# Dunni3/keypoint-diffusion

Measured on AMD Instinct MI355X. Metric: denoising steps/sec, higher is better.
Workload: dtype f32; 1 GPU; egnn_all_atom dynamics (6 EGNN layers, hidden 256, update_kp_feat; fixed receptor encoder), batch of 64 synthetic 300-atom pockets / 25-atom ligands per GPU, T=500, seeded random-init weights, every step taken from the t=T ligand state; batch_per_gpu=64, n_rec=300, n_lig=25, parallelism=dp1

## Files before the change

### keypoint-diffusion_amd/csrc/egnn.hip

```cpp
#include <string.h>

#include <map>
#include <set>
#include <string>
#include <vector>

#include "egnn_kernels.h"
#include "egnn_wide.h"
#include "mfma_core.h"

using namespace kpd;

namespace {

struct LayerW {
    float *wp_e[4], *wx_e[4], *b_e[4], *wr_e[4], *watt[4];
    float *wp_c[4], *wx_c[4], *b_c[4], *wr_c[4], *w3[4];
    void *wh_e[4], *wh_c[4];
    void *chh_p[2][NSLOT];
    void *wh_a[2], *wh_b[2], *wh_2[2];
    float *wp_p[2][NSLOT], *wx_p[2][NSLOT], *b_p[2][NSLOT];
    float *ch_p[2][NSLOT], *wcol_p[2][NSLOT];
    float *wp_a[2], *wx_a[2], *wp_b[2], *wx_b[2], *b0[2], *wp_2[2], *wx_2[2], *b2[2], *ln_w[2], *ln_b[2];
};

const int kSrcNt[4] = {NT_LIG, NT_KP, NT_LIG, NT_KP};
const int kDstNt[4] = {NT_LIG, NT_LIG, NT_KP, NT_KP};
const int kSrcSlot[4] = {0, 0, 6, 4};
const int kDstSlot[4] = {2, 4, 2, 6};
const char *kEtName[4] = {"ll", "kl", "lk", "kk"};
const char *kNtName[2] = {"lig", "kp"};

std::vector<std::string> split(const std::string &s, char c) {
    std::vector<std::string> out;
    size_t p = 0;
    while (true) {
        size_t q = s.find(c, p);
        out.push_back(s.substr(p, q == std::string::npos ? q : q - p));
        if (q == std::string::npos) break;
        p = q + 1;
    }
    return out;
}

int et_index(const std::string &s) {
    for (int i = 0; i < 4; ++i)
        if (s == kEtName[i]) return i;
    return -1;
}
int nt_index(const std::string &s) {
    for (int i = 0; i < 2; ++i)
        if (s == kNtName[i]) return i;
    return -1;
}

}

struct kpd_egnn {
    kpd_egnn_config cfg;
    int n_et;
    int n_upd;
    bool rec_identity;
    Arena warena, ws;
    std::vector<LayerW> L;
    float *le_W0, *le_b0, *le_W1t, *le_b1;
    float *re_W0, *re_b0, *re_W1t, *re_b1;
    float *de_W0, *de_b0, *de_W1, *de_b1;
    std::set<std::string> expected, loaded;
    bool committed = false;
    int debug_layers = -1;
    bool f16_ok = true;
    float *widen_buf = nullptr;
    int *widen_map = nullptr;
    size_t widen_floats = 0, widen_ints = 0;
    int gemm_mode = 0;
    bool f32_only = false;
    int prune_last = 1;
    bool prof_on = false;
    std::vector<hipEvent_t> prof_ev;
    size_t prof_used = 0;

    int cap_B = 0, cap_lig = 0, cap_kp = 0, cap_kk = 0, cap_ll = 0, cap_kl = 0, cap_maxlig = 0, cap_maxkp = 0;
    int tile_cap = 0, tiles_et_cap[4] = {0, 0, 0, 0};
    float *h[2], *x[2], *P[2];
    float *hn_main[4], *hn_cont[4], *xn_main[4], *xn_cont[4];
    int *bidx[2];
    float *z[2];
    int *meta, *ll_deg, *ll_off, *kl_off, *kl_pg;
    kpd_lig_graph lg;
    EgnnWide *wide = nullptr;
};

static kpd_status build_weight_arena(kpd_egnn *m) {
    const kpd_egnn_config &c = m->cfg;
    m->warena.poison_at = 2;
    m->L.assign(c.n_layers, LayerW());
    return carve(m->warena, ARENA_TAIL, [&](Carve &A) {
        for (int i = 0; i < c.n_layers; ++i) {
            LayerW &w = m->L[i];
            const std::string pre = "egnn.conv_layers." + std::to_string(i) + ".";
            for (int et = 0; et < m->n_et; ++et) {
                A(w.wp_e[et], WP_FLOATS); A(w.wx_e[et], HS); A(w.b_e[et], HS); A(w.wr_e[et], HS); A(w.watt[et], HS);
                A(w.wp_c[et], WP_FLOATS); A(w.wx_c[et], HS); A(w.b_c[et], HS); A(w.wr_c[et], HS); A(w.w3[et], HS);
                A.as<unsigned short>(w.wh_e[et], WH_HALVES); A.as<unsigned short>(w.wh_c[et], WH_HALVES);
                for (int var = 0; var < 2; ++var) {
                    const int ss = kSrcSlot[et] + var, ds = kDstSlot[et] + var;
                    A(w.wp_p[kSrcNt[et]][ss], WP_FLOATS); A(w.wx_p[kSrcNt[et]][ss], HS);
                    A(w.wp_p[kDstNt[et]][ds], WP_FLOATS); A(w.wx_p[kDstNt[et]][ds], HS); A(w.b_p[kDstNt[et]][ds], HS);
                    A(w.ch_p[kSrcNt[et]][ss], 16 * 4096); A(w.wcol_p[kSrcNt[et]][ss], HS);
                    A(w.ch_p[kDstNt[et]][ds], 16 * 4096); A(w.wcol_p[kDstNt[et]][ds], HS);
                    A.as<unsigned short>(w.chh_p[kSrcNt[et]][ss], CHH_HALVES);
                    A.as<unsigned short>(w.chh_p[kDstNt[et]][ds], CHH_HALVES);
                }
                const std::string e = kEtName[et];
                for (const char *blk : {"edge_mlp.", "coord_mlp."})
                    for (const char *s : {".0.weight", ".0.bias", ".2.weight", ".2.bias"}) m->expected.insert(pre + blk + e + s);
                m->expected.insert(pre + "coord_mlp." + e + ".4.weight");
                m->expected.insert(pre + "soft_attention." + e + ".0.weight");
                m->expected.insert(pre + "soft_attention." + e + ".0.bias");
            }
            for (int nt = 0; nt < m->n_upd; ++nt) {
                A(w.wp_a[nt], WP_FLOATS); A(w.wx_a[nt], HS); A(w.wp_b[nt], WP_FLOATS); A(w.wx_b[nt], HS); A(w.b0[nt], HS);
                A(w.wp_2[nt], WP_FLOATS); A(w.wx_2[nt], HS); A(w.b2[nt], HS); A(w.ln_w[nt], HS); A(w.ln_b[nt], HS);
                A.as<unsigned short>(w.wh_a[nt], WH_HALVES); A.as<unsigned short>(w.wh_b[nt], WH_HALVES);
                A.as<unsigned short>(w.wh_2[nt], WH_HALVES);
                const std::string n = kNtName[nt];
                for (const char *s : {".0.weight", ".0.bias", ".2.weight", ".2.bias"}) m->expected.insert(pre + "node_mlp." + n + s);
                if (c.norm) {
                    m->expected.insert(pre + "layer_norm." + n + ".weight");
                    m->expected.insert(pre + "layer_norm." + n + ".bias");
// ... 468 lines not shown
        ea.use_tanh = c.use_tanh; ea.coords_range = c.coords_range;
        ea.tile_rows = tr;
        ea.gemm_mode = tr == TM ? m->gemm_mode : 0;
        for (int et = 0; et < 4; ++et) {
            ea.src[et] = esrc[et]; ea.dst[et] = edst[et];
            ea.src_nt[et] = kSrcNt[et]; ea.dst_nt[et] = kDstNt[et]; ea.src_slot[et] = kSrcSlot[et]; ea.dst_slot[et] = kDstSlot[et];
            ea.wr_e[et] = L.wr_e[et]; ea.wr_c[et] = L.wr_c[et];
            ea.wp_e[et] = L.wp_e[et]; ea.wx_e[et] = L.wx_e[et]; ea.b_e[et] = L.b_e[et];
            ea.wp_c[et] = L.wp_c[et]; ea.wx_c[et] = L.wx_c[et]; ea.b_c[et] = L.b_c[et];
            ea.wh_e[et] = L.wh_e[et]; ea.wh_c[et] = L.wh_c[et];
            ea.watt[et] = L.watt[et]; ea.w3[et] = L.w3[et];
            ea.hn_main[et] = m->hn_main[et]; ea.hn_cont[et] = m->hn_cont[et];
            ea.xn_main[et] = m->xn_main[et]; ea.xn_cont[et] = m->xn_cont[et];
        }
        const bool prof = m->prof_on && m->prof_used + 2 <= m->prof_ev.size();
        if (prof) KPD_HIP(hipEventRecord(m->prof_ev[m->prof_used], st));
        KPD_TRY(launch_egnn_edge(ea, last ? tile_cap_last : tile_cap, st));
        if (prof) {
            KPD_HIP(hipEventRecord(m->prof_ev[m->prof_used + 1], st));
            m->prof_used += 2;
        }
        auto fill_update = [&](NodeArgs &na, int nt) {
            na.n = n[nt]; na.h = m->h[nt]; na.x = m->x[nt]; na.bidx = m->bidx[nt]; na.z = m->z[nt];
            int k = 0;
            for (int et = 0; et < m->n_et; ++et)
                if (kDstNt[et] == nt && ((layer_etmask(li) >> et) & 1)) {
                    na.rowptr[k] = rowptr[et];
                    na.hn_main[k] = m->hn_main[et]; na.hn_cont[k] = m->hn_cont[et];
                    na.xn_main[k] = m->xn_main[et]; na.xn_cont[k] = m->xn_cont[et];
                    ++k;
                }
            na.n_in = k;
            na.wp_a = L.wp_a[nt]; na.wx_a = L.wx_a[nt]; na.wp_b = L.wp_b[nt]; na.wx_b = L.wx_b[nt]; na.b0 = L.b0[nt];
            na.wp_2 = L.wp_2[nt]; na.wx_2 = L.wx_2[nt]; na.b2 = L.b2[nt]; na.ln_w = L.ln_w[nt]; na.ln_b = L.ln_b[nt];
            na.ln_inv_n = 1.0f / (float)(c.hidden_nf + 1); na.ln_pad = (float)(HID - c.hidden_nf);
            na.wh_a = L.wh_a[nt]; na.wh_b = L.wh_b[nt]; na.wh_2 = L.wh_2[nt];
            na.norm = c.norm;
            na.tile_shift = 6;
        };
        {
            NodeLayerPair lp;
            memset(&lp, 0, sizeof(lp));
            for (int nt = 0; nt < 2; ++nt) {
                NodeLayerArgs &na = lp.nt[nt];
                na.u.n = n[nt]; na.u.h = m->h[nt];
                if (nt < m->n_upd && !(nt == NT_KP && last && prune)) {
                    fill_update(na.u, nt);
                    na.do_update = 1;
                }
                if (!na.do_update && !na.do_proj) na.u.n = 0;
            }
            lp.tiles0 = cdiv(lp.nt[0].u.n, TN);
            lp.gemm_mode = m->gemm_mode;
            KPD_TRY(launch_node_layer(lp, st));
        }
    }
    KPD_TRY(launch_decode(m->h[NT_LIG], m->x[NT_LIG], bt->lig_x, bt->n_lig, c.atom_nf, 2 * c.atom_nf, m->de_W0, m->de_b0,
                          m->de_W1, m->de_b1, eps_h, eps_x, st));
    return KPD_OK;
}

extern "C" kpd_status kpd_egnn_debug_state(kpd_egnn *m, const char *what, float *out, int64_t n_floats, void *stream) {
    KPD_REQUIRE(m && what && out, KPD_ERR_INVALID, "null argument");
    hipStream_t st = static_cast<hipStream_t>(stream);
    if (m->wide) return wide_debug_state(m->wide, what, out, n_floats, st);
    const std::string w(what);
    const float *src = nullptr;
    if (w == "h_lig") src = m->h[0];
    else if (w == "h_kp") src = m->h[1];
    else if (w == "x_lig") src = m->x[0];
    else if (w == "x_kp") src = m->x[1];
    else if (w == "z_lig") src = m->z[0];
    else if (w == "z_kp") src = m->z[1];
    else if (w.size() == 4 && (w.rfind("xnm", 0) == 0 || w.rfind("xnc", 0) == 0 || w.rfind("hnm", 0) == 0 || w.rfind("hnc", 0) == 0) &&
             w[3] >= '0' && w[3] < '4') {
        const int et = w[3] - '0';
        src = w[0] == 'x' ? (w[2] == 'm' ? m->xn_main[et] : m->xn_cont[et]) : (w[2] == 'm' ? m->hn_main[et] : m->hn_cont[et]);
    }
    else if (w.rfind("layers=", 0) == 0) {
        m->debug_layers = atoi(w.c_str() + 7);
        return KPD_OK;
    } else if (w.rfind("prune=", 0) == 0) {
        m->prune_last = atoi(w.c_str() + 6);
        return KPD_OK;
    } else if (w.rfind("gemm=", 0) == 0) {
        const std::string v = w.substr(5);
        KPD_REQUIRE(v == "f32" || v == "f16x2", KPD_ERR_INVALID, "gemm mode must be f32 or f16x2");
        KPD_REQUIRE(v == "f32" || !m->f32_only, KPD_ERR_INVALID,
                    "gemm=f16x2: atom_nf = %d / rec_nf = %d (hidden_nf = %d) run the exact fp32 path only; the f16x2 mode covers atom_nf <= 32 "
                    "with rec_nf <= 128 or 256, or the identity keypoint encoder at hidden_nf 256", m->cfg.atom_nf, m->cfg.rec_nf, m->cfg.hidden_nf);
        KPD_REQUIRE(v == "f32" || !m->committed || m->f16_ok, KPD_ERR_WEIGHTS, "%s", F16_RANGE_ERROR);
        m->gemm_mode = v == "f16x2" ? 1 : 0;
        return KPD_OK;
    }
    KPD_REQUIRE(src, KPD_ERR_INVALID, "unknown debug tap '%s'", what);
    KPD_HIP(hipMemcpyAsync(out, src, (size_t)n_floats * 4, hipMemcpyDeviceToDevice, st));
    return KPD_OK;
}

extern "C" kpd_status kpd_egnn_profile(kpd_egnn *m, int32_t enable) {
    KPD_REQUIRE(m, KPD_ERR_INVALID, "null handle");
    KPD_REQUIRE(!m->wide, KPD_ERR_INVALID, "kpd_egnn_profile times the fused edge kernel of hidden_nf <= 256; hidden_nf = %d has none",
                m->cfg.hidden_nf);
    if (enable && m->prof_ev.empty()) {
        m->prof_ev.resize(2 * 8192);
        for (hipEvent_t &e : m->prof_ev) KPD_HIP(hipEventCreate(&e));
    }
    m->prof_on = enable != 0;
    m->prof_used = 0;
    return KPD_OK;
}

extern "C" kpd_status kpd_egnn_profile_read(kpd_egnn *m, double *total_ms, int32_t *launches) {
    KPD_REQUIRE(m && total_ms && launches, KPD_ERR_INVALID, "null argument");
    KPD_REQUIRE(!m->wide, KPD_ERR_INVALID, "kpd_egnn_profile_read: no fused edge kernel at hidden_nf = %d", m->cfg.hidden_nf);
    double tot = 0.0;
    for (size_t i = 0; i + 1 < m->prof_used; i += 2) {
        KPD_HIP(hipEventSynchronize(m->prof_ev[i + 1]));
        float ms = 0.0f;
        KPD_HIP(hipEventElapsedTime(&ms, m->prof_ev[i], m->prof_ev[i + 1]));
        tot += ms;
    }
    *total_ms = tot;
    *launches = (int32_t)(m->prof_used / 2);
    return KPD_OK;
}

extern "C" kpd_status kpd_egnn_last_counts(kpd_egnn *m, int32_t out[8], void *stream) {
    KPD_REQUIRE(m && out, KPD_ERR_INVALID, "null argument");
    if (m->wide) return wide_last_counts(m->wide, out, static_cast<hipStream_t>(stream));
    for (int i = 0; i < 7; ++i) out[i] = 0;
    out[7] = m->gemm_mode;
    if (!m->ws.base) return KPD_OK;
    hipStream_t st = static_cast<hipStream_t>(stream);
    int host[25];
    KPD_HIP(hipMemcpyAsync(host, m->meta, sizeof(host), hipMemcpyDeviceToHost, st));
    KPD_HIP(hipStreamSynchronize(st));
// ... 23 lines not shown
```

### keypoint-diffusion_amd/csrc/egnn_kernels.h

```cpp
#pragma once
#include "engine.h"

namespace kpd {

constexpr int NSLOT = 8;
constexpr int ATT_BIAS_AT = 260;
constexpr int BIAS_K = 260;
constexpr int ET_LL = 0, ET_KL = 1, ET_LK = 2, ET_KK = 3;
constexpr int NT_LIG = 0, NT_KP = 1;

constexpr int EDGE_LDS_BYTES = TM * SA * 4 + (TM * 2 + TM + 3 * TM + TM + 3 * TM + 4 * HS + 8 + TM) * 4;
constexpr int EDGE_H_LDS_BYTES = 64 * 280 * 2 * 2 + (TM * 2 + TM + 3 * TM + TM + 3 * TM + 2 * HS + 8) * 4 + 2 * 2 * 272 * 2;

struct ProjArgs {
    const float *h;
    int n;
    float *P;
    const float *wp[NSLOT];
    const float *wx[NSLOT];
    const float *bias[NSLOT];
    int slot[NSLOT];
    const float *chain[NSLOT];
    const float *wcol[NSLOT];
    const void *chain_h[NSLOT];
// ... 58 lines not shown
};

struct EdgeBwdArgs {
    const int *meta;
    const int *dst[4];
    int dst_nt[4];
    const float *dhn[2];
    const float *dxo[2];
    const float *zinv[2];
    float *keep[4][2][4];
    float *att[4], *sc[4], *nvec[4];
    const float *dij[4];
    const float *wa[4], *w3[4];
    const float *wpT[4][2], *wxT[4][2], *wr[4][2];
    float *dv_main[4][2], *dv_cont[4][2], *dvw_main[4][2], *dvw_cont[4][2];
    float *part[2];
    int part_ld;
    int use_tanh;
    float coords_range;
};

struct NodeArgs {
    int n;
    float *h;
    float *x;
    const int *bidx;
    const float *z;
    int n_in;
    const int *rowptr[2];
    const float *hn_main[2], *hn_cont[2];
    const float *xn_main[2], *xn_cont[2];
    const float *wp_a, *wx_a, *wp_b, *wx_b, *b0;
    const float *wp_2, *wx_2, *b2;
    const void *wh_a, *wh_b, *wh_2;
    const float *ln_w, *ln_b;
    int norm;
    float ln_inv_n, ln_pad;
    int tile_shift;
};

struct NodeLayerArgs {
    NodeArgs u;
    int do_update, do_proj;
    float *P;
    int n_slots;
    const float *wp[NSLOT], *wx[NSLOT], *bias[NSLOT];
    int slot[NSLOT];
};

struct NodeLayerPair {
    NodeLayerArgs nt[2];
    int tiles0;
    int gemm_mode;
};

constexpr int TN = 32;
constexpr int NODE_LAYER_LDS_BYTES = TN * SA * 4 + 3 * TN * 4 + 3 * HS * 4;
constexpr int NODE_H_TILE_FLOATS = 2 * TN * 280 / 2;
constexpr int NODE_H_LDS_BYTES = NODE_H_TILE_FLOATS * 4 + 3 * TN * 4;


kpd_status egnn_kernels_init();
kpd_status launch_node_graph_index(const int *ptr, int B, int n, int *bidx, hipStream_t st);
kpd_status launch_egnn_meta(const int *counts, int e_kk, int active_mask, int active_last, const int *lig_ptr, const int *kp_ptr,
                            const int *ll_per_graph, const int *kk_rowptr, int B, const int *kl_off, float message_norm,
                            int update_kp, int *meta, float *z_lig, float *z_kp, hipStream_t st, int tile_rows = TM);
kpd_status launch_embed(const float *in, int n, int fin, const float *W0, const float *b0, int hid, const float *W1t,
                        const float *b1, const float *t, const int *bidx, float *out, int identity, hipStream_t st);
kpd_status launch_decode(const float *h, const float *x, const float *x0, int n, int atom_nf, int hid, const float *W0,
                         const float *b0, const float *W1, const float *b1, float *eps_h, float *eps_x, hipStream_t st);
kpd_status launch_egnn_edge(const EdgeArgs &a, int tile_cap, hipStream_t st);
kpd_status launch_egnn_edge_train(const EdgeTrainArgs &a, int tile_cap, hipStream_t st);
struct EdgePiecesSumArgs {
    const float *hn_main[4], *hn_cont[4], *xn_main[4], *xn_cont[4];
    const int *rowptr[4];
    int live[4], dst_nt[4];
    const float *zinv[2];
    int n[2];
    float *hn[2], *xn[2];
};
kpd_status launch_edge_pieces_sum(const EdgePiecesSumArgs &a, hipStream_t st);
kpd_status launch_edge_train_pack(const EdgePackTab &t, hipStream_t st);
kpd_status launch_egnn_edge_bwd(const EdgeBwdArgs &a, int tile_cap, hipStream_t st);
struct EdgePiecesBatch {
    struct One {
        const float *m1, *c1, *m2, *c2;
        const int *rowptr;
        int n;
        float *o1, *o2;
    } e[8];
    int ldo;
};
kpd_status launch_edge_pieces_set(const EdgePiecesBatch &b, int count, hipStream_t st);
kpd_status launch_proj_chain(const ProjPair &p, hipStream_t st);
kpd_status launch_node_layer(const NodeLayerPair &p, hipStream_t st);

}
```

### keypoint-diffusion_amd/csrc/egnn_kernels.hip

```cpp
#include <stdlib.h>

#include <algorithm>

#include "egnn_kernels.h"
#include "mfma_core.h"

namespace kpd {

__global__ void k_node_graph_index(const int *__restrict__ ptr, int B, int n, int *__restrict__ bidx) {
    const int i = blockIdx.x * blockDim.x + threadIdx.x;
    if (i >= n) return;
    int lo = 0, hi = B;
    while (hi - lo > 1) {
        const int mid = (lo + hi) >> 1;
        if (ptr[mid] <= i) lo = mid; else hi = mid;
    }
    bidx[i] = lo;
}

__global__ void k_egnn_meta(const int *__restrict__ counts, int e_kk, int active_mask, int active_last, const int *__restrict__ lig_ptr,
                            const int *__restrict__ kp_ptr, const int *__restrict__ ll_per_graph,
                            const int *__restrict__ kk_rowptr, int B, const int *__restrict__ kl_off, float message_norm,
                            int update_kp, int tile_rows, int *__restrict__ meta, float *__restrict__ z_lig, float *__restrict__ z_kp) {
    if (blockIdx.x == 0 && threadIdx.x < 2) {
// ... 1341 lines not shown
    lds_barrier();

    edge_gather_finish_h<NW>(gc, s, Ah, a.wr_c[et], wave, lane);
    lds_barrier();
    acc_zero_w<NW>(acc);
    ex = row_dot_h2<TPR>(Ah, wxs + 544, tid);
    if constexpr (NW == 4) gemm_rows64_h(Ah, a.wh_c[et], acc, wave, lane);
    else gemm_rows64_h8(Ah, a.wh_c[et], acc, wave, lane);
    unscale_acc(acc, ex);
    lds_barrier();
    store_T_silu_w<NW, true>(s.A, acc, ex, a.b_c[et], tid, wave, lane);
    lds_barrier();
    {
        float dot = row_dot_chunks<TPR>(s.A, s.wv + HS, 64, tid);
        const int row = tid / TPR;
        if ((tid % TPR) == 0) {
            dot = fmaf(s.A[row * SA + 256], s.wv[HS + 256], dot);
            float c = a.use_tanh ? tanhf(dot) * a.coords_range : dot;
            if (row >= ne) c = 0.0f;
            s.mx[3 * row] = c * s.xd[3 * row];
            s.mx[3 * row + 1] = c * s.xd[3 * row + 1];
            s.mx[3 * row + 2] = c * s.xd[3 * row + 2];
        }
    }
    lds_barrier();
    if (wave == 0) {
        const unsigned long long heads =
            ((unsigned long long)(unsigned)s.misc[5] << 32) | (unsigned long long)(unsigned)s.misc[4];
        const unsigned long long upto = lane == 63 ? ~0ull : ((1ull << (lane + 1)) - 1ull);
        const int start = 63 - __clzll((long long)((heads & upto) | 1ull));
        float vx = s.mx[3 * lane], vy = s.mx[3 * lane + 1], vz = s.mx[3 * lane + 2];
#pragma unroll
        for (int off = 1; off < 64; off <<= 1) {
            const float tx = __shfl_up(vx, off), ty = __shfl_up(vy, off), tz = __shfl_up(vz, off);
            if (lane - off >= start) {
                vx += tx;
                vy += ty;
                vz += tz;
            }
        }
        if ((endmask >> lane) & 1ull) {
            const int piece = __popcll(endmask & ((1ull << lane) - 1ull));
            float *out = (piece == 0 && first_is_cont) ? a.xn_cont[et] + (size_t)tile_in_et * 4
                                                       : a.xn_main[et] + (size_t)((unsigned)s.dst[lane] / PROW_B) * 4;
            out[0] = vx;
            out[1] = vy;
            out[2] = vz;
        }
    }
}



__global__ __launch_bounds__(512) __attribute__((amdgpu_waves_per_eu(6, 6))) void k_node_update8(NodeLayerPair p) {
    extern __shared__ __attribute__((aligned(16))) float smem[];
    float *A = smem;
    float *s_z = smem + TN * SA;
    float *s_mean = s_z + TN;
    float *s_rstd = s_mean + TN;
    float *s_wx = s_rstd + TN;
    const int tid = threadIdx.x, wave = __builtin_amdgcn_readfirstlane(tid >> 6), lane = tid & 63;
    const int which = blockIdx.x >= p.tiles0 ? 1 : 0;
    const NodeLayerArgs &L = p.nt[which];
    const NodeArgs &a = L.u;
    const int node0 = (blockIdx.x - (which ? p.tiles0 : 0)) * TN;
    constexpr int RPW = TN / 8;
    constexpr int TPR = 512 / TN;

    auto load_h = [&]() {
        f32x4 val[RPW], val2[RPW];
#pragma unroll
        for (int rr = 0; rr < RPW; ++rr) {
            const f32x4 *src = reinterpret_cast<const f32x4 *>(a.h + (size_t)(node0 + wave * RPW + rr) * HS);
            val[rr] = src[lane];
            val2[rr] = src[64 + (lane & 1)];
        }
#pragma unroll
        for (int rr = 0; rr < RPW; ++rr) {
            const int r = wave * RPW + rr;
            *reinterpret_cast<f32x4 *>(A + r * SA + 4 * lane) = val[rr];
            if (lane < 2) *reinterpret_cast<f32x4 *>(A + r * SA + 256 + 4 * lane) = val2[rr];
        }
    };
    const int two = a.n_in > 1 ? 1 : 0;
    const int *__restrict__ rp0 = a.rowptr[0], *__restrict__ rp1 = a.rowptr[two];

    f32x16 acc;
    {
        if (tid < TN) {
            const int v = node0 + tid;
            float z = 1.0f;
            if (v < a.n) {
                const int lo0 = rp0[v], hi0 = rp0[v + 1], lo1 = rp1[v], hi1 = two ? rp1[v + 1] : lo1;
                const float *pm0 = a.xn_main[0] + (size_t)v * 4, *pm1 = a.xn_main[two] + (size_t)v * 4;
                const float m0x = pm0[0], m0y = pm0[1], m0z = pm0[2], m1x = pm1[0], m1y = pm1[1], m1z = pm1[2];
                z = a.z[a.bidx[v]];
                float sx = 0.f, sy = 0.f, sz = 0.f;
                if (hi0 > lo0) {
                    sx += m0x; sy += m0y; sz += m0z;
                    for (int t = (lo0 >> a.tile_shift) + 1; t <= ((hi0 - 1) >> a.tile_shift); ++t) {
                        const float *q = a.xn_cont[0] + (size_t)t * 4;
                        sx += q[0]; sy += q[1]; sz += q[2];
                    }
                }
                if (hi1 > lo1) {
                    sx += m1x; sy += m1y; sz += m1z;
                    for (int t = (lo1 >> a.tile_shift) + 1; t <= ((hi1 - 1) >> a.tile_shift); ++t) {
                        const float *q = a.xn_cont[two] + (size_t)t * 4;
                        sx += q[0]; sy += q[1]; sz += q[2];
                    }
                }
                float *xv = a.x + (size_t)v * 3;
                xv[0] += sx / z; xv[1] += sy / z; xv[2] += sz / z;
            }
            s_z[tid] = z;
        } else if (tid >= 512 - 3 * 66) {
            const int i = tid - (512 - 3 * 66), which = i / 66, j = i - which * 66;
            const float *row = which == 0 ? a.wx_a : which == 1 ? a.wx_b : a.wx_2;
            reinterpret_cast<f32x4 *>(s_wx + which * HS)[j] = reinterpret_cast<const f32x4 *>(row)[j];
        }
        load_h();
        lds_barrier();
#pragma unroll
        for (int i = 0; i < 16; ++i) acc[i] = 0.0f;
        gemm_rows32_t8<NG, SA>(A, a.wp_a, acc, wave, lane);
        float ex = row_dot_chunks<TPR>(A, s_wx, KP / 4, tid);
        lds_barrier();
        {
            constexpr int GB = 2;
#pragma unroll
            for (int r0 = 0; r0 < RPW; r0 += GB) {
                int lo0[GB], hi0[GB], lo1[GB], hi1[GB];
                f32x4 m0[GB], m1[GB];
                float t0[GB], t1[GB];
#pragma unroll
                for (int rr = 0; rr < GB; ++rr) {
                    const int v = min(node0 + wave * RPW + r0 + rr, a.n - 1);
                    lo0[rr] = rp0[v]; hi0[rr] = rp0[v + 1];
                    lo1[rr] = rp1[v]; hi1[rr] = two ? rp1[v + 1] : lo1[rr];
                    const f32x4 *p0 = reinterpret_cast<const f32x4 *>(a.hn_main[0] + (size_t)v * HS);
                    const f32x4 *p1 = reinterpret_cast<const f32x4 *>(a.hn_main[two] + (size_t)v * HS);
                    m0[rr] = p0[lane]; t0[rr] = reinterpret_cast<const float *>(p0)[256 + (lane & 7)];
                    m1[rr] = p1[lane]; t1[rr] = reinterpret_cast<const float *>(p1)[256 + (lane & 7)];
                }
#pragma unroll
                for (int rr = 0; rr < GB; ++rr) {
                    const int r = wave * RPW + r0 + rr, v = node0 + r;
                    f32x4 val = {0.f, 0.f, 0.f, 0.f};
                    float val2 = 0.0f;
                    if (v < a.n) {
                        if (hi0[rr] > lo0[rr]) {
                            val += m0[rr];
                            val2 += t0[rr];
                            for (int t = (lo0[rr] >> a.tile_shift) + 1; t <= ((hi0[rr] - 1) >> a.tile_shift); ++t) {
                                const f32x4 *q = reinterpret_cast<const f32x4 *>(a.hn_cont[0] + (size_t)t * HS);
                                val += q[lane];
                                val2 += reinterpret_cast<const float *>(q)[256 + (lane & 7)];
                            }
                        }
                        if (hi1[rr] > lo1[rr]) {
                            val += m1[rr];
                            val2 += t1[rr];
                            for (int t = (lo1[rr] >> a.tile_shift) + 1; t <= ((hi1[rr] - 1) >> a.tile_shift); ++t) {
                                const f32x4 *q = reinterpret_cast<const f32x4 *>(a.hn_cont[two] + (size_t)t * HS);
                                val += q[lane];
                                val2 += reinterpret_cast<const float *>(q)[256 + (lane & 7)];
                            }
                        }
                        const float z = s_z[r];
                        val /= z;
                        val2 /= z;
                    }
                    *reinterpret_cast<f32x4 *>(A + r * SA + 4 * lane) = val;
                    if (lane < 8) A[r * SA + 256 + lane] = val2;
                }
            }
        }
        lds_barrier();
        gemm_rows32_t8<NG, SA>(A, a.wp_b, acc, wave, lane);
        ex += row_dot_chunks<TPR>(A, s_wx + HS, KP / 4, tid);
        lds_barrier();
        {
            const int col = 32 * wave + (lane & 31);
            const float bb = a.b0[col];
#pragma unroll
            for (int reg = 0; reg < 16; ++reg) A[acc_row32(reg, lane) * SA + col] = silu(acc[reg] + bb);
        }
        if ((tid % TPR) == 0) A[(tid / TPR) * SA + 256] = silu(ex + a.b0[256]);
        lds_barrier();
#pragma unroll
        for (int i = 0; i < 16; ++i) acc[i] = 0.0f;
        gemm_rows32_t8<NG, SA>(A, a.wp_2, acc, wave, lane);
        ex = row_dot_chunks<TPR>(A, s_wx + 2 * HS, KP / 4, tid);
        lds_barrier();
        {
            const int col = 32 * wave + (lane & 31);
            const float bb = a.b2[col];
#pragma unroll
            for (int reg = 0; reg < 16; ++reg) A[acc_row32(reg, lane) * SA + col] = acc[reg] + bb;
        }
        if ((tid % TPR) == 0) A[(tid / TPR) * SA + 256] = ex + a.b2[256];
        lds_barrier();
#pragma unroll 4
        for (int rr = 0; rr < RPW; ++rr) {
            const int r = wave * RPW + rr;
            const f32x4 *src = reinterpret_cast<const f32x4 *>(a.h + (size_t)(node0 + r) * HS);
            *reinterpret_cast<f32x4 *>(A + r * SA + 4 * lane) += src[lane];
            if (lane == 0) A[r * SA + 256] += a.h[(size_t)(node0 + r) * HS + 256];
        }
        lds_barrier();
        if (a.norm) {
            const int row = tid / TPR, q = tid % TPR;
            const float *tr = A + row * SA + q;
            float sum = 0.0f;
            for (int i = 0; i < 256 / TPR; ++i) sum += tr[TPR * i];
            if (q == 0) sum += A[row * SA + 256];
#pragma unroll
            for (int o = 1; o < TPR; o <<= 1) sum += __shfl_xor(sum, o);
            const float mean = sum * a.ln_inv_n;
            float var = 0.0f;
            for (int i = 0; i < 256 / TPR; ++i) {
                const float dlt = tr[TPR * i] - mean;
                var = fmaf(dlt, dlt, var);
            }
            if (q == 0) {
                const float dlt = A[row * SA + 256] - mean;
                var = fmaf(dlt, dlt, var);
            }
#pragma unroll
            for (int o = 1; o < TPR; o <<= 1) var += __shfl_xor(var, o);
            if (q == 0) {
                s_mean[row] = mean;
                s_rstd[row] = 1.0f / sqrtf((var - a.ln_pad * mean * mean) * a.ln_inv_n + 1e-5f);
            }
        }
        lds_barrier();
#pragma unroll 2
        for (int rr = 0; rr < RPW; ++rr) {
            const int r = wave * RPW + rr, v = node0 + r;
            f32x4 val = *reinterpret_cast<const f32x4 *>(A + r * SA + 4 * lane);
            float last = A[r * SA + 256];
            if (a.norm) {
                const float mean = s_mean[r], rstd = s_rstd[r];
                const f32x4 w = reinterpret_cast<const f32x4 *>(a.ln_w)[lane];
                const f32x4 b = reinterpret_cast<const f32x4 *>(a.ln_b)[lane];
                val = (val - mean) * rstd * w + b;
                last = (last - mean) * rstd * a.ln_w[256] + a.ln_b[256];
            }
            if (v >= a.n) {
                val = f32x4{0.f, 0.f, 0.f, 0.f};
                last = 0.0f;
            }
            *reinterpret_cast<f32x4 *>(A + r * SA + 4 * lane) = val;
            const f32x4 t = {last, 0.f, 0.f, 0.f};
            if (lane == 0) *reinterpret_cast<f32x4 *>(A + r * SA + 256) = t;
            if (lane == 1) *reinterpret_cast<f32x4 *>(A + r * SA + 260) = f32x4{0.f, 0.f, 0.f, 0.f};
            if (v < a.n) {
                f32x4 *dst = reinterpret_cast<f32x4 *>(a.h + (size_t)v * HS);
                dst[lane] = val;
                if (lane == 0) dst[64] = t;
            }
        }
        lds_barrier();
    }
}


__global__ __launch_bounds__(512) __attribute__((amdgpu_waves_per_eu(4, 6))) void k_node_update8_h(NodeLayerPair p) {
    extern __shared__ __attribute__((aligned(16))) float smem[];
    float *A = smem;
    _Float16 *Ah = reinterpret_cast<_Float16 *>(smem);
    constexpr int PN = TN * SAH;
    float *s_z = smem + NODE_H_TILE_FLOATS;
    float *s_mean = s_z + TN;
    float *s_rstd = s_mean + TN;
    const int tid = threadIdx.x, wave = tid >> 6, lane = tid & 63;
    const int which = blockIdx.x >= p.tiles0 ? 1 : 0;
    const NodeLayerArgs &L = p.nt[which];
    const NodeArgs &a = L.u;
    const int node0 = (blockIdx.x - (which ? p.tiles0 : 0)) * TN;
    constexpr int RPW = TN / 8;
    constexpr int TPR = 512 / TN;
    typedef unsigned u32x2 __attribute__((ext_vector_type(2)));

    auto put_row = [&](int r, const f32x4 &val, const f32x4 &val2) {
        unsigned h0, h1, l0, l1;
        split_pair(H_SCALE_A * val[0], H_SCALE_A * val[1], h0, l0);
        split_pair(H_SCALE_A * val[2], H_SCALE_A * val[3], h1, l1);
        *reinterpret_cast<u32x2 *>(Ah + r * SAH + 4 * lane) = u32x2{h0, h1};
        *reinterpret_cast<u32x2 *>(Ah + PN + r * SAH + 4 * lane) = u32x2{l0, l1};
        if (lane < 4) {
            split_pair(H_SCALE_A * val2[0], H_SCALE_A * val2[1], h0, l0);
            split_pair(H_SCALE_A * val2[2], H_SCALE_A * val2[3], h1, l1);
            *reinterpret_cast<u32x2 *>(Ah + r * SAH + 256 + 4 * lane) = u32x2{h0, h1};
            *reinterpret_cast<u32x2 *>(Ah + PN + r * SAH + 256 + 4 * lane) = u32x2{l0, l1};
        }
    };
    auto put_elem = [&](int row, int col, float v) {
        const float sv = H_SCALE_A * v;
        const _Float16 hi = (_Float16)sv;
        Ah[row * SAH + col] = hi;
        Ah[PN + row * SAH + col] = (_Float16)(sv - (float)hi);
    };

    f32x16 acc;
    if (tid < TN) {
        const int v = node0 + tid;
        float z = 1.0f;
        if (v < a.n) {
            z = a.z[a.bidx[v]];
            float sx = 0.f, sy = 0.f, sz = 0.f;
            for (int i = 0; i < a.n_in; ++i) {
                const int lo = a.rowptr[i][v], hi = a.rowptr[i][v + 1];
                if (hi > lo) {
                    const float *pm = a.xn_main[i] + (size_t)v * 4;
                    sx += pm[0]; sy += pm[1]; sz += pm[2];
// ... 166 lines not shown
    if (n == 0) return KPD_OK;
    KPD_REQUIRE(hid <= 512 && atom_nf <= 256, KPD_ERR_INVALID, "decode: hid=%d atom_nf=%d exceed 512 / 256", hid, atom_nf);
    if (hid <= 64 && atom_nf <= 64)
        hipLaunchKernelGGL(k_decode<64>, dim3(n), dim3(64), 0, st, h, x, x0, n, atom_nf, hid, W0, b0, W1, b1, eps_h, eps_x);
    else
        hipLaunchKernelGGL(k_decode<512>, dim3(n), dim3(64), 0, st, h, x, x0, n, atom_nf, hid, W0, b0, W1, b1, eps_h, eps_x);
    KPD_LAUNCH_CHECK();
    return KPD_OK;
}

kpd_status launch_egnn_edge(const EdgeArgs &a, int tile_cap, hipStream_t st) {
    if (tile_cap == 0) return KPD_OK;
    if (poison_level() >= 1) KPD_TRY(poison_lds(st));
    KPD_REQUIRE(a.tile_rows == TM, KPD_ERR_INVALID, "the edge kernels walk 64-edge tiles");
    if (a.gemm_mode == 1) {
        for (int et = 0; et < 4; ++et)
            KPD_REQUIRE(!a.wp_e[et] || (a.wh_e[et] && a.wh_c[et]), KPD_ERR_STATE, "f16x2 weights of edge type %d were not packed", et);
        KPD_TRY(ensure_dynamic_lds(reinterpret_cast<const void *>(k_egnn_edge_h<4>), EDGE_H_LDS_BYTES));
        hipLaunchKernelGGL(k_egnn_edge_h<4>, dim3(8 * cdiv(tile_cap, 8)), dim3(256), EDGE_H_LDS_BYTES, st, a);
        KPD_LAUNCH_CHECK();
        return KPD_OK;
    }
    KPD_TRY(ensure_dynamic_lds(reinterpret_cast<const void *>(k_egnn_edge<4>), EDGE_LDS_BYTES));
    EdgeArgs b = a;
    b.split_slots = 2 * cu_count() / 8;
    hipLaunchKernelGGL(k_egnn_edge<4>, dim3(8 * (cdiv(tile_cap, 8) + b.split_slots / 2)), dim3(256), EDGE_LDS_BYTES, st, b);
    KPD_LAUNCH_CHECK();
    return KPD_OK;
}

kpd_status launch_node_layer(const NodeLayerPair &p, hipStream_t st) {
    const int tiles = p.tiles0 + cdiv(p.nt[1].u.n, TN);
    if (tiles == 0) return KPD_OK;
    if (poison_level() >= 1) KPD_TRY(poison_lds(st));
    for (int nt = 0; nt < 2; ++nt)
        KPD_REQUIRE(p.nt[nt].u.n == 0 || (p.nt[nt].do_update && !p.nt[nt].do_proj), KPD_ERR_INVALID, "node launch: update-only node types expected");
    for (int nt = 0; nt < 2; ++nt) {
        const NodeArgs &u = p.nt[nt].u;
        if (u.n == 0) continue;
        KPD_REQUIRE(u.n_in >= 1 && u.n_in <= 2, KPD_ERR_INVALID, "node launch: node type %d has %d incoming edge types (1 or 2 expected)", nt, u.n_in);
        for (int i = 0; i < u.n_in; ++i)
            KPD_REQUIRE(u.rowptr[i] && u.hn_main[i] && u.hn_cont[i] && u.xn_main[i] && u.xn_cont[i], KPD_ERR_INVALID,
                        "node launch: segment arrays of incoming edge type %d of node type %d are missing", i, nt);
    }
    if (p.gemm_mode == 1) {
        for (int nt = 0; nt < 2; ++nt)
            if (p.nt[nt].u.n > 0)
                KPD_REQUIRE(p.nt[nt].u.wh_a && p.nt[nt].u.wh_b && p.nt[nt].u.wh_2, KPD_ERR_STATE, "node weights of type %d have no f16 planes", nt);
        KPD_TRY(ensure_dynamic_lds(reinterpret_cast<const void *>(k_node_update8_h), NODE_H_LDS_BYTES));
        hipLaunchKernelGGL(k_node_update8_h, dim3(tiles), dim3(512), NODE_H_LDS_BYTES, st, p);
        KPD_LAUNCH_CHECK();
        return KPD_OK;
    }
    KPD_TRY(ensure_dynamic_lds(reinterpret_cast<const void *>(k_node_update8), NODE_LAYER_LDS_BYTES));
    hipLaunchKernelGGL(k_node_update8, dim3(tiles), dim3(512), NODE_LAYER_LDS_BYTES, st, p);
    KPD_LAUNCH_CHECK();
    return KPD_OK;
}


kpd_status launch_egnn_edge_train(const EdgeTrainArgs &a, int tile_cap, hipStream_t st) {
    if (tile_cap == 0) return KPD_OK;
    KPD_TRY(ensure_dynamic_lds(reinterpret_cast<const void *>(k_egnn_edge_train), EDGE_LDS_BYTES));
    hipLaunchKernelGGL(k_egnn_edge_train, dim3(8 * cdiv(tile_cap, 8)), dim3(256), EDGE_LDS_BYTES, st, a);
    KPD_LAUNCH_CHECK();
    return KPD_OK;
}

kpd_status launch_edge_pieces_sum(const EdgePiecesSumArgs &a, hipStream_t st) {
    const int most = std::max(a.n[0], a.n[1]);
    if (most == 0) return KPD_OK;
    hipLaunchKernelGGL(k_edge_pieces_sum, dim3(cdiv(most, 4), 2), dim3(256), 0, st, a);
    KPD_LAUNCH_CHECK();
    return KPD_OK;
}

kpd_status launch_egnn_edge_bwd(const EdgeBwdArgs &a, int tile_cap, hipStream_t st) {
    if (tile_cap == 0) return KPD_OK;
    KPD_TRY(ensure_dynamic_lds(reinterpret_cast<const void *>(k_egnn_edge_bwd), EDGE_BWD_LDS_BYTES));
    hipLaunchKernelGGL(k_egnn_edge_bwd, dim3(8 * cdiv(tile_cap, 8)), dim3(256), EDGE_BWD_LDS_BYTES, st, a);
    KPD_LAUNCH_CHECK();
    return KPD_OK;
}

kpd_status launch_edge_pieces_set(const EdgePiecesBatch &b, int count, hipStream_t st) {
    int most = 0;
    for (int i = 0; i < count; ++i) most = std::max(most, b.e[i].n);
    if (count == 0 || most == 0) return KPD_OK;
    KPD_REQUIRE(count <= 8, KPD_ERR_INVALID, "edge pieces: %d pairs in one launch (at most 8)", count);
    hipLaunchKernelGGL(k_edge_pieces_set, dim3(cdiv(most, 4), count), dim3(256), 0, st, b);
    KPD_LAUNCH_CHECK();
    return KPD_OK;
}

kpd_status launch_edge_train_pack(const EdgePackTab &t, hipStream_t st) {
    if (t.n == 0) return KPD_OK;
    hipLaunchKernelGGL(k_edge_train_pack, dim3(cdiv(WP_FLOATS + 3 * HS, 256), t.n), dim3(256), 0, st, t);
    KPD_LAUNCH_CHECK();
    return KPD_OK;
}

}
```

### keypoint-diffusion_amd/csrc/mfma_core.h

```cpp
#pragma once
#include "common.h"

namespace kpd {

typedef float f32x16 __attribute__((ext_vector_type(16)));
typedef float f32x4 __attribute__((ext_vector_type(4)));

__device__ __forceinline__ float silu(float x) { return x * __builtin_amdgcn_rcpf(1.0f + __expf(-x)); }
constexpr float SILU_C = -1.4426950408889634f;
__device__ __forceinline__ float silu_pre(float xs) { return xs * __builtin_amdgcn_rcpf(1.0f + __builtin_amdgcn_exp2f(xs)); }
typedef float silu_f32x4 __attribute__((ext_vector_type(4)));
__device__ __forceinline__ silu_f32x4 silu_pre4(silu_f32x4 v) {
    const silu_f32x4 q = {__builtin_amdgcn_rcpf(1.0f + __builtin_amdgcn_exp2f(v[0])), __builtin_amdgcn_rcpf(1.0f + __builtin_amdgcn_exp2f(v[1])),
                          __builtin_amdgcn_rcpf(1.0f + __builtin_amdgcn_exp2f(v[2])), __builtin_amdgcn_rcpf(1.0f + __builtin_amdgcn_exp2f(v[3]))};
    return v * q;
}
__device__ __forceinline__ float sigmoidf_(float x) { return __builtin_amdgcn_rcpf(1.0f + __expf(-x)); }

__device__ __forceinline__ void acc_zero(f32x16 (&acc)[2][2]) {
#pragma unroll
    for (int m = 0; m < 2; ++m)
#pragma unroll
        for (int n = 0; n < 2; ++n)
#pragma unroll
// ... 148 lines not shown
            __builtin_amdgcn_sched_barrier(0);
            const int gn = g + 4 + i < NG_ ? g + 4 + i : NG_ - 1;
            KPD_LOAD32(i, gn)
        }
    }
    static_assert((NG_ & 3) <= 1, "tail handling assumes at most one group past the last quad");
    if (NG_ & 3) {
        __builtin_amdgcn_sched_barrier(0);
#pragma unroll
        for (int j = 0; j < TailSteps<NG_>::J; ++j) {
            acc[0] = __builtin_amdgcn_mfma_f32_32x32x2f32(a0[0][j], b0[0][j], acc[0], 0, 0, 0);
            acc[1] = __builtin_amdgcn_mfma_f32_32x32x2f32(a0[0][j], b1[0][j], acc[1], 0, 0, 0);
        }
    }
#undef KPD_LOAD32
#undef KPD_STEP32
}

template <int NG_, int SA_>
__device__ __forceinline__ void gemm_rows32_t8(const float *__restrict__ A, const float *__restrict__ Wp, f32x16 &acc, int wave,
                                               int lane) {
    const int r = lane & 31, h = lane >> 5;
    const float *a0p = A + r * SA_ + 4 * h;
    const f32x4 *bp = reinterpret_cast<const f32x4 *>(Wp) + ((wave >> 1) * 64 + lane) * 2 + (wave & 1);
    f32x4 a0[4], b0[4];
#define KPD_LOAD32(S, G)                                     \
    a0[S] = *reinterpret_cast<const f32x4 *>(a0p + 8 * (G)); \
    b0[S] = bp[(G) * 512];
#define KPD_STEP32(S) \
    _Pragma("unroll") for (int j = 0; j < 4; ++j) acc = __builtin_amdgcn_mfma_f32_32x32x2f32(a0[S][j], b0[S][j], acc, 0, 0, 0);
#pragma unroll
    for (int i = 0; i < 4; ++i) {
        const int g = i < NG_ ? i : NG_ - 1;
        KPD_LOAD32(i, g)
    }
    constexpr int QUADS = NG_ / 4;
#pragma unroll 1
    for (int q = 0; q < QUADS; ++q) {
        const int g = 4 * q;
#pragma unroll
        for (int i = 0; i < 4; ++i) {
            __builtin_amdgcn_sched_barrier(0);
            KPD_STEP32(i)
            __builtin_amdgcn_sched_barrier(0);
            const int gn = g + 4 + i < NG_ ? g + 4 + i : NG_ - 1;
            KPD_LOAD32(i, gn)
        }
    }
    static_assert((NG_ & 3) <= 1, "tail handling assumes at most one group past the last quad");
    if (NG_ & 3) {
        __builtin_amdgcn_sched_barrier(0);
#pragma unroll
        for (int j = 0; j < TailSteps<NG_>::J; ++j) acc = __builtin_amdgcn_mfma_f32_32x32x2f32(a0[0][j], b0[0][j], acc, 0, 0, 0);
    }
#undef KPD_LOAD32
#undef KPD_STEP32
}

__device__ __forceinline__ int acc_row32(int reg, int lane) { return (reg & 3) + 8 * (reg >> 2) + 4 * (lane >> 5); }

template <int NW>
struct WaveCols {
    static constexpr int NT = 8 / NW;
};

template <int NW>
__device__ __forceinline__ void acc_zero_w(f32x16 (&acc)[2][WaveCols<NW>::NT]) {
#pragma unroll
    for (int m = 0; m < 2; ++m)
#pragma unroll
        for (int n = 0; n < WaveCols<NW>::NT; ++n)
#pragma unroll
            for (int r = 0; r < 16; ++r) acc[m][n][r] = 0.0f;
}

template <int NW>
__device__ __forceinline__ int acc_col_w(int nt, int wave, int lane) {
    return NW == 4 ? 64 * wave + 32 * nt + (lane & 31) : 32 * wave + (lane & 31);
}

template <int NW, int NG_, int SA_>
__device__ __forceinline__ void gemm_rows64_w(const float *__restrict__ A, const float *__restrict__ Wp,
                                              f32x16 (&acc)[2][WaveCols<NW>::NT], int wave, int lane) {
    if constexpr (NW == 4) {
        gemm_rows64_t<NG_, SA_>(A, Wp, acc, wave, lane);
    } else {
        const int r = lane & 31, h = lane >> 5;
        const float *a0p = A + r * SA_ + 4 * h;
        const float *a1p = A + (32 + r) * SA_ + 4 * h;
        const f32x4 *bp = reinterpret_cast<const f32x4 *>(Wp) + ((wave >> 1) * 64 + lane) * 2 + (wave & 1);
        f32x4 xa0, xa1, xb0, ya0, ya1, yb0;
#define KPD_LOAD1(A0, A1, B0, G)                                      \
    A0 = *reinterpret_cast<const f32x4 *>(a0p + 8 * (G));             \
    A1 = *reinterpret_cast<const f32x4 *>(a1p + 8 * (G));             \
    B0 = bp[(G) * 512];
#define KPD_STEP1(A0, A1, B0)                                                                     \
    _Pragma("unroll") for (int j = 0; j < 4; ++j) {                                               \
        acc[0][0] = __builtin_amdgcn_mfma_f32_32x32x2f32(A0[j], B0[j], acc[0][0], 0, 0, 0);       \
        acc[1][0] = __builtin_amdgcn_mfma_f32_32x32x2f32(A1[j], B0[j], acc[1][0], 0, 0, 0);       \
    }
        KPD_LOAD1(xa0, xa1, xb0, 0)
        if (NG_ > 1) {
            KPD_LOAD1(ya0, ya1, yb0, 1)
        }
        constexpr int PAIRS = NG_ / 2;
#pragma unroll 1
// ... 267 lines not shown
```

Baseline: 153.0 steps/s.

## Pair node-update tiles per workgroup when tile count exceeds CU count

Node update kernel is templated to process one or two 32-row tiles per workgroup. A new 2-tile GEMM shares each weight fetch across both tiles. A host-side plan picks how many tile pairs to use from the CU count, so the grid shrinks to about one wave of workgroups when there are more tiles than CUs. The pair path doubles LDS per block and lowers the waves_per_eu hint from 6 to 4. The trailing LDS zero-fill of padded rows and the final barrier are dropped.

```diff
diff --git a/keypoint-diffusion_amd/csrc/egnn.hip b/keypoint-diffusion_amd/csrc/egnn.hip
--- a/keypoint-diffusion_amd/csrc/egnn.hip
+++ b/keypoint-diffusion_amd/csrc/egnn.hip
@@ -76,6 +76,7 @@
     int gemm_mode = 0;
     bool f32_only = false;
     int prune_last = 1;
+    int node_cus = 0;
     bool prof_on = false;
     std::vector<hipEvent_t> prof_ev;
     size_t prof_used = 0;
@@ -650,6 +651,7 @@
             }
             lp.tiles0 = cdiv(lp.nt[0].u.n, TN);
             lp.gemm_mode = m->gemm_mode;
+            lp.plan_cus = m->node_cus;
             KPD_TRY(launch_node_layer(lp, st));
         }
     }
@@ -681,6 +683,10 @@
     } else if (w.rfind("prune=", 0) == 0) {
         m->prune_last = atoi(w.c_str() + 6);
         return KPD_OK;
+    } else if (w.rfind("node_cus=", 0) == 0) {
+        m->node_cus = atoi(w.c_str() + 9);
+        KPD_REQUIRE(m->node_cus >= 0, KPD_ERR_INVALID, "node_cus must be >= 0");
+        return KPD_OK;
     } else if (w.rfind("gemm=", 0) == 0) {
         const std::string v = w.substr(5);
         KPD_REQUIRE(v == "f32" || v == "f16x2", KPD_ERR_INVALID, "gemm mode must be f32 or f16x2");
diff --git a/keypoint-diffusion_amd/csrc/egnn_kernels.h b/keypoint-diffusion_amd/csrc/egnn_kernels.h
--- a/keypoint-diffusion_amd/csrc/egnn_kernels.h
+++ b/keypoint-diffusion_amd/csrc/egnn_kernels.h
@@ -134,10 +134,28 @@
     NodeLayerArgs nt[2];
     int tiles0;
     int gemm_mode;
+    int plan_cus;
+    int pairs[2];
 };
 
 constexpr int TN = 32;
-constexpr int NODE_LAYER_LDS_BYTES = TN * SA * 4 + 3 * TN * 4 + 3 * HS * 4;
+constexpr int node_layer_lds_bytes(int tiles_per_wg) { return tiles_per_wg * (TN * SA * 4 + 3 * TN * 4) + 3 * HS * 4; }
+constexpr int NODE_LAYER_LDS_BYTES = node_layer_lds_bytes(2);
+
+struct NodePairPlan {
+    int pairs[2];
+};
+inline NodePairPlan node_pair_plan(int tiles0, int tiles1, int cus) {
+    NodePairPlan plan = {{0, 0}};
+    const int tiles = tiles0 + tiles1;
+    if (cus <= 0 || tiles <= cus) return plan;
+    const long long m = ((long long)tiles + cus - 1) / cus;
+    const long long slots = (long long)cus * (m / 2);
+    plan.pairs[0] = (int)(tiles0 / 2 < slots ? tiles0 / 2 : slots);
+    const long long rest = slots - plan.pairs[0];
+    plan.pairs[1] = (int)(tiles1 / 2 < rest ? tiles1 / 2 : rest);
+    return plan;
+}
 constexpr int NODE_H_TILE_FLOATS = 2 * TN * 280 / 2;
 constexpr int NODE_H_LDS_BYTES = NODE_H_TILE_FLOATS * 4 + 3 * TN * 4;
 
diff --git a/keypoint-diffusion_amd/csrc/egnn_kernels.hip b/keypoint-diffusion_amd/csrc/egnn_kernels.hip
--- a/keypoint-diffusion_amd/csrc/egnn_kernels.hip
+++ b/keypoint-diffusion_amd/csrc/egnn_kernels.hip
@@ -1417,19 +1417,16 @@
 
 
 
-__global__ __launch_bounds__(512) __attribute__((amdgpu_waves_per_eu(6, 6))) void k_node_update8(NodeLayerPair p) {
-    extern __shared__ __attribute__((aligned(16))) float smem[];
+template <int NTL>
+__device__ __forceinline__ void node_update_tiles(const NodeArgs &a, const int node0, float *smem, const int tid, const int wave,
+                                                  const int lane) {
+    constexpr int ROWS = NTL * TN;
     float *A = smem;
-    float *s_z = smem + TN * SA;
-    float *s_mean = s_z + TN;
-    float *s_rstd = s_mean + TN;
-    float *s_wx = s_rstd + TN;
-    const int tid = threadIdx.x, wave = __builtin_amdgcn_readfirstlane(tid >> 6), lane = tid & 63;
-    const int which = blockIdx.x >= p.tiles0 ? 1 : 0;
-    const NodeLayerArgs &L = p.nt[which];
-    const NodeArgs &a = L.u;
-    const int node0 = (blockIdx.x - (which ? p.tiles0 : 0)) * TN;
-    constexpr int RPW = TN / 8;
+    float *s_z = smem + ROWS * SA;
+    float *s_mean = s_z + ROWS;
+    float *s_rstd = s_mean + ROWS;
+    float *s_wx = s_rstd + ROWS;
+    constexpr int RPW = ROWS / 8;
     constexpr int TPR = 512 / TN;
 
     auto load_h = [&]() {
@@ -1447,12 +1444,17 @@
             if (lane < 2) *reinterpret_cast<f32x4 *>(A + r * SA + 256 + 4 * lane) = val2[rr];
         }
     };
+    auto gemm = [&](const float *__restrict__ Wp, f32x16 (&acc)[NTL]) {
+        if constexpr (NTL == 1) gemm_rows32_t8<NG, SA>(A, Wp, acc[0], wave, lane);
+        else gemm_rows32x2_t8<NG, SA>(A, Wp, acc, wave, lane);
+    };
     const int two = a.n_in > 1 ? 1 : 0;
     const int *__restrict__ rp0 = a.rowptr[0], *__restrict__ rp1 = a.rowptr[two];
 
-    f32x16 acc;
+    f32x16 acc[NTL];
+    float ex[NTL];
     {
-        if (tid < TN) {
+        if (tid < ROWS) {
             const int v = node0 + tid;
             float z = 1.0f;
             if (v < a.n) {
@@ -1487,12 +1489,15 @@
         load_h();
         lds_barrier();
 #pragma unroll
-        for (int i = 0; i < 16; ++i) acc[i] = 0.0f;
-        gemm_rows32_t8<NG, SA>(A, a.wp_a, acc, wave, lane);
-        float ex = row_dot_chunks<TPR>(A, s_wx, KP / 4, tid);
+        for (int t = 0; t < NTL; ++t)
+#pragma unroll
+            for (int i = 0; i < 16; ++i) acc[t][i] = 0.0f;
+        gemm(a.wp_a, acc);
+#pragma unroll
+        for (int t = 0; t < NTL; ++t) ex[t] = row_dot_chunks<TPR>(A + t * TN * SA, s_wx, KP / 4, tid);
         lds_barrier();
         {
-            constexpr int GB = 2;
+            constexpr int GB = 2 * NTL;
 #pragma unroll
             for (int r0 = 0; r0 < RPW; r0 += GB) {
                 int lo0[GB], hi0[GB], lo1[GB], hi1[GB];
@@ -1542,29 +1547,45 @@
             }
         }
         lds_barrier();
-        gemm_rows32_t8<NG, SA>(A, a.wp_b, acc, wave, lane);
-        ex += row_dot_chunks<TPR>(A, s_wx + HS, KP / 4, tid);
+        gemm(a.wp_b, acc);
+#pragma unroll
+        for (int t = 0; t < NTL; ++t) ex[t] += row_dot_chunks<TPR>(A + t * TN * SA, s_wx + HS, KP / 4, tid);
         lds_barrier();
         {
             const int col = 32 * wave + (lane & 31);
             const float bb = a.b0[col];
 #pragma unroll
-            for (int reg = 0; reg < 16; ++reg) A[acc_row32(reg, lane) * SA + col] = silu(acc[reg] + bb);
-        }
-        if ((tid % TPR) == 0) A[(tid / TPR) * SA + 256] = silu(ex + a.b0[256]);
+            for (int t = 0; t < NTL; ++t)
+#pragma unroll
+                for (int reg = 0; reg < 16; ++reg) A[(t * TN + acc_row32(reg, lane)) * SA + col] = silu(acc[t][reg] + bb);
+        }
+        if ((tid % TPR) == 0) {
+            const float bb = a.b0[256];
+#pragma unroll
+            for (int t = 0; t < NTL; ++t) A[(t * TN + tid / TPR) * SA + 256] = silu(ex[t] + bb);
+        }
         lds_barrier();
 #pragma unroll
-        for (int i = 0; i < 16; ++i) acc[i] = 0.0f;
-        gemm_rows32_t8<NG, SA>(A, a.wp_2, acc, wave, lane);
-        ex = row_dot_chunks<TPR>(A, s_wx + 2 * HS, KP / 4, tid);
+        for (int t = 0; t < NTL; ++t)
+#pragma unroll
+            for (int i = 0; i < 16; ++i) acc[t][i] = 0.0f;
+        gemm(a.wp_2, acc);
+#pragma unroll
+        for (int t = 0; t < NTL; ++t) ex[t] = row_dot_chunks<TPR>(A + t * TN * SA, s_wx + 2 * HS, KP / 4, tid);
         lds_barrier();
         {
             const int col = 32 * wave + (lane & 31);
             const float bb = a.b2[col];
 #pragma unroll
-            for (int reg = 0; reg < 16; ++reg) A[acc_row32(reg, lane) * SA + col] = acc[reg] + bb;
-        }
-        if ((tid % TPR) == 0) A[(tid / TPR) * SA + 256] = ex + a.b2[256];
+            for (int t = 0; t < NTL; ++t)
+#pragma unroll
+                for (int reg = 0; reg < 16; ++reg) A[(t * TN + acc_row32(reg, lane)) * SA + col] = acc[t][reg] + bb;
+        }
+        if ((tid % TPR) == 0) {
+            const float bb = a.b2[256];
+#pragma unroll
+            for (int t = 0; t < NTL; ++t) A[(t * TN + tid / TPR) * SA + 256] = ex[t] + bb;
+        }
         lds_barrier();
 #pragma unroll 4
         for (int rr = 0; rr < RPW; ++rr) {
@@ -1575,28 +1596,31 @@
         }
         lds_barrier();
         if (a.norm) {
-            const int row = tid / TPR, q = tid % TPR;
-            const float *tr = A + row * SA + q;
-            float sum = 0.0f;
-            for (int i = 0; i < 256 / TPR; ++i) sum += tr[TPR * i];
-            if (q == 0) sum += A[row * SA + 256];
-#pragma unroll
-            for (int o = 1; o < TPR; o <<= 1) sum += __shfl_xor(sum, o);
-            const float mean = sum * a.ln_inv_n;
-            float var = 0.0f;
-            for (int i = 0; i < 256 / TPR; ++i) {
-                const float dlt = tr[TPR * i] - mean;
-                var = fmaf(dlt, dlt, var);
-            }
-            if (q == 0) {
-                const float dlt = A[row * SA + 256] - mean;
-                var = fmaf(dlt, dlt, var);
-            }
-#pragma unroll
-            for (int o = 1; o < TPR; o <<= 1) var += __shfl_xor(var, o);
-            if (q == 0) {
-                s_mean[row] = mean;
-                s_rstd[row] = 1.0f / sqrtf((var - a.ln_pad * mean * mean) * a.ln_inv_n + 1e-5f);
+#pragma unroll
+            for (int t = 0; t < NTL; ++t) {
+                const int row = t * TN + tid / TPR, q = tid % TPR;
+                const float *tr = A + row * SA + q;
+                float sum = 0.0f;
+                for (int i = 0; i < 256 / TPR; ++i) sum += tr[TPR * i];
+                if (q == 0) sum += A[row * SA + 256];
+#pragma unroll
+                for (int o = 1; o < TPR; o <<= 1) sum += __shfl_xor(sum, o);
+                const float mean = sum * a.ln_inv_n;
+                float var = 0.0f;
+                for (int i = 0; i < 256 / TPR; ++i) {
+                    const float dlt = tr[TPR * i] - mean;
+                    var = fmaf(dlt, dlt, var);
+                }
+                if (q == 0) {
+                    const float dlt = A[row * SA + 256] - mean;
+                    var = fmaf(dlt, dlt, var);
+                }
+#pragma unroll
+                for (int o = 1; o < TPR; o <<= 1) var += __shfl_xor(var, o);
+                if (q == 0) {
+                    s_mean[row] = mean;
+                    s_rstd[row] = 1.0f / sqrtf((var - a.ln_pad * mean * mean) * a.ln_inv_n + 1e-5f);
+                }
             }
         }
         lds_barrier();
@@ -1612,21 +1636,30 @@
                 val = (val - mean) * rstd * w + b;
                 last = (last - mean) * rstd * a.ln_w[256] + a.ln_b[256];
             }
-            if (v >= a.n) {
-                val = f32x4{0.f, 0.f, 0.f, 0.f};
-                last = 0.0f;
-            }
-            *reinterpret_cast<f32x4 *>(A + r * SA + 4 * lane) = val;
-            const f32x4 t = {last, 0.f, 0.f, 0.f};
-            if (lane == 0) *reinterpret_cast<f32x4 *>(A + r * SA + 256) = t;
-            if (lane == 1) *reinterpret_cast<f32x4 *>(A + r * SA + 260) = f32x4{0.f, 0.f, 0.f, 0.f};
             if (v < a.n) {
                 f32x4 *dst = reinterpret_cast<f32x4 *>(a.h + (size_t)v * HS);
+                const f32x4 t = {last, 0.f, 0.f, 0.f};
                 dst[lane] = val;
                 if (lane == 0) dst[64] = t;
             }
         }
-        lds_barrier();
+    }
+}
+
+__global__ __launch_bounds__(512) __attribute__((amdgpu_waves_per_eu(4, 4))) void k_node_update8(NodeLayerPair p) {
+    extern __shared__ __attribute__((aligned(16))) float smem[];
+    const int tid = threadIdx.x, wave = __builtin_amdgcn_readfirstlane(tid >> 6), lane = tid & 63;
+    const int n_pairs = p.pairs[0] + p.pairs[1];
+    int b = blockIdx.x;
+    if (b < n_pairs) {
+        const int which = b >= p.pairs[0] ? 1 : 0;
+        node_update_tiles<2>(p.nt[which].u, (b - (which ? p.pairs[0] : 0)) * 2 * TN, smem, tid, wave, lane);
+    } else {
+        b -= n_pairs;
+        const int singles0 = p.tiles0 - 2 * p.pairs[0];
+        const int which = b >= singles0 ? 1 : 0;
+        const int tile = which ? 2 * p.pairs[1] + (b - singles0) : 2 * p.pairs[0] + b;
+        node_update_tiles<1>(p.nt[which].u, tile * TN, smem, tid, wave, lane);
     }
 }
 
@@ -1899,8 +1932,13 @@
         KPD_LAUNCH_CHECK();
         return KPD_OK;
     }
+    NodeLayerPair q = p;
+    const NodePairPlan plan = node_pair_plan(p.tiles0, tiles - p.tiles0, p.plan_cus > 0 ? p.plan_cus : cu_count());
+    q.pairs[0] = plan.pairs[0];
+    q.pairs[1] = plan.pairs[1];
+    const int n_pairs = plan.pairs[0] + plan.pairs[1];
     KPD_TRY(ensure_dynamic_lds(reinterpret_cast<const void *>(k_node_update8), NODE_LAYER_LDS_BYTES));
-    hipLaunchKernelGGL(k_node_update8, dim3(tiles), dim3(512), NODE_LAYER_LDS_BYTES, st, p);
+    hipLaunchKernelGGL(k_node_update8, dim3(tiles - n_pairs), dim3(512), node_layer_lds_bytes(n_pairs ? 2 : 1), st, q);
     KPD_LAUNCH_CHECK();
     return KPD_OK;
 }
diff --git a/keypoint-diffusion_amd/csrc/mfma_core.h b/keypoint-diffusion_amd/csrc/mfma_core.h
--- a/keypoint-diffusion_amd/csrc/mfma_core.h
+++ b/keypoint-diffusion_amd/csrc/mfma_core.h
@@ -224,6 +224,54 @@
         __builtin_amdgcn_sched_barrier(0);
 #pragma unroll
         for (int j = 0; j < TailSteps<NG_>::J; ++j) acc = __builtin_amdgcn_mfma_f32_32x32x2f32(a0[0][j], b0[0][j], acc, 0, 0, 0);
+    }
+#undef KPD_LOAD32
+#undef KPD_STEP32
+}
+
+template <int NG_, int SA_>
+__device__ __forceinline__ void gemm_rows32x2_t8(const float *__restrict__ A, const float *__restrict__ Wp, f32x16 (&acc)[2], int wave,
+                                                 int lane) {
+    const int r = lane & 31, h = lane >> 5;
+    const float *a0p = A + r * SA_ + 4 * h;
+    const float *a1p = a0p + 32 * SA_;
+    const f32x4 *bp = reinterpret_cast<const f32x4 *>(Wp) + ((wave >> 1) * 64 + lane) * 2 + (wave & 1);
+    f32x4 a0[4], a1[4], b0[4];
+#define KPD_LOAD32(S, G)                                     \
+    a0[S] = *reinterpret_cast<const f32x4 *>(a0p + 8 * (G)); \
+    a1[S] = *reinterpret_cast<const f32x4 *>(a1p + 8 * (G)); \
+    b0[S] = bp[(G) * 512];
+#define KPD_STEP32(S)                                                                          \
+    _Pragma("unroll") for (int j = 0; j < 4; ++j) {                                            \
+        acc[0] = __builtin_amdgcn_mfma_f32_32x32x2f32(a0[S][j], b0[S][j], acc[0], 0, 0, 0);    \
+        acc[1] = __builtin_amdgcn_mfma_f32_32x32x2f32(a1[S][j], b0[S][j], acc[1], 0, 0, 0);    \
+    }
+#pragma unroll
+    for (int i = 0; i < 4; ++i) {
+        const int g = i < NG_ ? i : NG_ - 1;
+        KPD_LOAD32(i, g)
+    }
+    constexpr int QUADS = NG_ / 4;
+#pragma unroll 1
+    for (int q = 0; q < QUADS; ++q) {
+        const int g = 4 * q;
+#pragma unroll
+        for (int i = 0; i < 4; ++i) {
+            __builtin_amdgcn_sched_barrier(0);
+            KPD_STEP32(i)
+            __builtin_amdgcn_sched_barrier(0);
+            const int gn = g + 4 + i < NG_ ? g + 4 + i : NG_ - 1;
+            KPD_LOAD32(i, gn)
+        }
+    }
+    static_assert((NG_ & 3) <= 1, "tail handling assumes at most one group past the last quad");
+    if (NG_ & 3) {
+        __builtin_amdgcn_sched_barrier(0);
+#pragma unroll
+        for (int j = 0; j < TailSteps<NG_>::J; ++j) {
+            acc[0] = __builtin_amdgcn_mfma_f32_32x32x2f32(a0[0][j], b0[0][j], acc[0], 0, 0, 0);
+            acc[1] = __builtin_amdgcn_mfma_f32_32x32x2f32(a1[0][j], b0[0][j], acc[1], 0, 0, 0);
+        }
     }
 #undef KPD_LOAD32
 #undef KPD_STEP32
```

Result: no change. 153.2 steps/s, median of 6 (+0.1%).
